# HopperLogger/HopperRender

Measured on AMD Instinct MI355X. Metric: interpolated frames/sec + ms/flow-calc, 2160p HDR, 1/2/4/8 MI355X, higher is better.
Workload: dtype u16

## Files before the change

### hopperrender_amd/csrc/hf_calc.hip

```cpp

#include "hf_ctx.h"

using namespace hfi;

namespace hfi {

int enqueue_flow_chain(const hf_ctx* const* cs, int n, hipStream_t s) {
    const hf_ctx* c = cs[0];
    const hf::Geom& g = c->g;
    const int iters = effective_iterations(c);
    bool any_big = false;
    for (int k = 0; k < iters; k++) any_big |= c->levels[k].window > 32;

    hf::FlowBatch a{};
    a.n = n;
    for (int i = 0; i < n; i++) {
        const hf_ctx* m = cs[i];
        hf::FlowStep& f = a.s[i];
        f.pp1 = m->pp[1].get();
        f.pp2 = m->pp[2].get();
        f.pl = m->pl;
        f.total_delta = m->d_total_delta;
        f.R = c->p.search_radius;
        f.delta_scalar = c->p.delta_scalar;
        f.neighbor_scalar = c->p.neighbor_scalar;
        f.delta_divisor = (uint32_t)(g.lh * g.lw * (g.hdr ? 6 : 10));
        f.sadtab = m->sadtab.get(); f.sad_nbx = m->sad_nbx; f.sad_nby = m->sad_nby;
        f.tables_base = m->tables.get(); f.sums_base = m->sums.get();
        f.counters = c->counters.get();
        f.still_count = m->still_count.get();
    }
    hf::FlowLevel none{};
    hf::PendingArgmin pending[hf::kMaxFlowBatch] = {};
    int step_index = 0;
    auto flush_pending = [&]() {
        if (!pending[0].active) return;
        hf::FlowBatch b = a;
        for (int i = 0; i < n; i++) {
            hf::FlowStep& f = b.s[i];
            const hf::PendingArgmin& p = pending[i];
            f.cur = p.lvl; f.prev = p.lvl_prev; f.axis = p.axis; f.capture_delta = p.capture_delta;
            f.sums = const_cast<uint32_t*>(p.sums); f.use_neighbors = p.use_neighbors; f.pend = hf::PendingArgmin{};
            pending[i] = hf::PendingArgmin{};
        }
        hf::launch_flow_big_argmin(g, b, s);
    };
    const bool lazy = !(c->cfg.flags & HF_FLAG_NO_LAZY_ARGMIN);
    bool tables_fresh = false;
    for (int k = 0; k < iters; k++) {
        const bool use_neighbors = k >= 4;
        if (use_neighbors) flush_pending();
        const bool small = c->levels[k].window <= 32;
        for (int axis = 0; axis < (small ? 1 : 2); axis++) {
            for (int i = 0; i < n; i++) {
                const hf_ctx* m = cs[i];
                hf::FlowStep& f = a.s[i];
                f.cur = m->levels[k];
                f.prev = k ? m->levels[k - 1] : none;
                f.prev2 = k > 1 ? m->levels[k - 2] : none;
                f.level_index = k;
                const hf::SadUse sad = hf::plan_sad_tables(m->levels.data(), k, c->tab_mode && m->sadtab);
                f.sad_write = sad.write; f.sad_read = sad.read;
                f.use_neighbors = use_neighbors;
                f.axis = axis;
                f.capture_delta = (k == 0 && axis == 0);
                f.pend = pending[i];
                if (!small) f.sums = m->sums.get() + (size_t)step_index * m->sums_stride;
                pending[i] = hf::PendingArgmin{};
            }
            if (a.s[0].sad_read && !tables_fresh)
                return fail(const_cast<hf_ctx*>(c), HF_ERR_STATE, "flow chain: level %d (window %d) would read SAD tables that level %d did not write", k, c->levels[k].window, k - 1);
            tables_fresh = a.s[0].sad_write != 0;
            if (small) {
                hf::launch_flow_level_small(g, a, s);
            } else {
                hf::launch_flow_big_partial(g, a, s);
                for (int i = 0; i < n; i++) {
                    const hf::FlowStep& f = a.s[i];
                    pending[i].active = 1; pending[i].axis = axis; pending[i].capture_delta = f.capture_delta;
                    pending[i].use_neighbors = f.use_neighbors;
                    pending[i].lvl = f.cur; pending[i].lvl_prev = f.prev; pending[i].sums = f.sums;
                }
                step_index++;
                if (!lazy || use_neighbors) flush_pending();
            }
        }
    }
    flush_pending();
    hf::BlurBatch bb{};
    bb.n = n;
    for (int i = 0; i < n; i++) {
        const hf_ctx* m = cs[i];
        bb.s[i].last = iters ? m->levels[iters - 1] : none;
        bb.s[i].blurred = m->blurred[0].get();
        bb.s[i].packed = m->blurred_xy[0].get();
        bb.s[i].zero = any_big ? m->sums.get() : nullptr;
        bb.s[i].still_count = m->still_count.get();
        bb.s[i].still_out = m->still_count ? m->d_total_delta + 1 : nullptr;
    }
    hf::launch_blur_flow(g, bb, c->cfg.blur_radius, (int)(c->sums_bytes / sizeof(uint32_t)), s);
    HF_HIP(const_cast<hf_ctx*>(c), hipGetLastError());
    return HF_OK;
}

bool choose_tab_mode(hf_ctx* const* cs, int n) {
    hf_ctx* l = cs[0];
    if (!l->sadtab) return false;
    if (l->cfg.flags & HF_FLAG_SAD_REUSE_ALWAYS) return true;
    if (n < 4) return false;
    float sum = 0.f;
    int have = 0;
    for (int i = 0; i < n; i++) {
        hf_ctx* m = cs[i];
        const uint32_t raw = m->h_total_delta ? ((volatile uint32_t*)m->h_total_delta.get())[1] : 0xFFFFFFFFu;
        int n32 = 0;
        for (const hf::FlowLevel& L : m->levels) if (L.window == 32) n32 = L.nwx * L.nwy;
        if (raw != 0xFFFFFFFFu && n32 > 0) {
            const float share = (float)raw / (float)n32;
            m->still_share = m->still_share < 0.f ? share : 0.5f * m->still_share + 0.5f * share;
        }
        if (m->still_share >= 0.f) { sum += m->still_share; have++; }
    }
    if (!have) return l->tab_mode;
    const float share = sum / (float)have;
    return l->tab_mode ? share >= 0.30f : share >= 0.45f;
// ... 450 lines not shown
```

### hopperrender_amd/csrc/hf_context.hip

```cpp

#include "hf_ctx.h"

using namespace hfi;

namespace {
thread_local std::string g_create_error;
}

namespace hfi {
std::shared_mutex g_capture_mutex;
std::atomic<int64_t> g_live[kLiveKinds];
}

namespace hfi {

int fail(hf_ctx* c, int code, const char* fmt, ...) {
    char buf[512];
    va_list ap;
    va_start(ap, fmt);
    vsnprintf(buf, sizeof(buf), fmt, ap);
    va_end(ap);
    std::string msg = std::string("[HopperRender] ") + buf;
    if (c) c->err = msg; else g_create_error = msg;
    return code;
// ... 149 lines not shown
    hf::Geom& g = c->g;
    g.hdr = cfg->is_hdr ? 1 : 0;
    g.H = cfg->frame_height;
    g.W = cfg->frame_width;
    g.in_stride = cfg->input_stride > 0 ? cfg->input_stride : g.W;
    g.out_stride = cfg->output_stride > 0 ? cfg->output_stride : g.W;
    g.rs = 0;
    while ((g.H >> g.rs) > cfg->max_calc_res) g.rs++;
    g.lw = (int)std::ceil((double)g.W / std::pow(2.0, g.rs));
    g.lh = (int)std::ceil((double)g.H / std::pow(2.0, g.rs));
    if (g.in_stride < g.W || g.out_stride < g.W) {
        delete c;
        return fail(nullptr, HF_ERR_INVALID_ARGUMENT, "hf_create: strides must be >= frame width");
    }
    if (((cfg->flags & HF_FLAG_PLANAR_IN) && (g.in_stride & 1)) || ((cfg->flags & HF_FLAG_PLANAR_OUT) && (g.out_stride & 1))) {
        delete c;
        return fail(nullptr, HF_ERR_INVALID_ARGUMENT, "hf_create: a planar side needs an even stride (input %d, output %d)", g.in_stride, g.out_stride);
    }
    if (c->cfg.blur_radius <= 0) c->cfg.blur_radius = 4;
    if (c->cfg.blur_radius > 64) { delete c; return fail(nullptr, HF_ERR_INVALID_ARGUMENT, "hf_create: blur_radius must be <= 64"); }
    c->p.delta_scalar = cfg->delta_scalar;
    c->p.neighbor_scalar = cfg->neighbor_scalar;
    c->p.black_level = cfg->black_level;
    c->p.white_level = cfg->white_level;
    c->p.search_radius = cfg->search_radius > 0 ? cfg->search_radius : kMinSearchRadius;
    c->p.frame_count = 0;
    if (c->p.search_radius < 2 || c->p.search_radius > kMaxSearchRadius) {
        delete c;
        return fail(nullptr, HF_ERR_INVALID_ARGUMENT, "hf_create: search_radius must be in [2, 16]");
    }

    const size_t bpp = g.hdr ? 2 : 1;
    c->in_bytes = bpp * ((size_t)g.H * g.in_stride + (size_t)(g.H / 2) * g.in_stride);
    c->out_bytes = bpp * ((size_t)g.H * g.out_stride + (size_t)(g.H / 2) * g.out_stride);
    c->plane_elems = (size_t)g.lw * g.lh;
    const int ws0 = initial_window(g.lw, g.lh);
    const int max_iters = ilog2(ws0);
    c->pl = hf::make_phase_layout(g, max_iters);
    {
        size_t elems = 0;
        for (int k = 0, w = ws0; k < max_iters; k++, w >>= 1) {
            hf::FlowLevel L{};
            L.window = w; L.log2w = ilog2(w);
            L.nwx = (g.lw + w - 1) / w; L.nwy = (g.lh + w - 1) / w;
            c->levels.push_back(L);
            elems += 2 * (size_t)L.nwx * L.nwy;
        }
        c->tables_bytes = (elems + 8) * sizeof(int16_t);
    }
    const size_t nwin_max = (size_t)((g.lw + 63) / 64) * ((g.lh + 63) / 64) + 1;
    c->sums_stride = nwin_max * 16;
    c->sums_bytes = (size_t)kMaxSteps * c->sums_stride * sizeof(uint32_t);
    c->sad_nbx = (g.lw + 1) / 2; c->sad_nby = (g.lh + 1) / 2;
    c->sadtab_bytes = (cfg->flags & HF_FLAG_NO_SAD_REUSE) ? 0 : 2 * (size_t)c->sad_nbx * c->sad_nby * 32;
    int rc = HF_OK;
    auto bail = [&](int code) { std::string e = c->err; hf_destroy(c); g_create_error = e; return code; };
    {
        const uint64_t required = 3 * c->in_bytes + 3 * c->pl.bytes + c->out_bytes + c->tables_bytes + c->sums_bytes + c->sadtab_bytes +
                                  2 * c->plane_elems * sizeof(int16_t) * 3 + 2 * c->plane_elems * sizeof(uint32_t);
        std::vector<hf_device_caps> caps((size_t)ndev);
        for (int d = 0; d < ndev; d++) {
            hipDeviceProp_t prop;
            if (hipGetDeviceProperties(&prop, d) != hipSuccess) { caps[(size_t)d] = hf_device_caps{}; continue; }
            caps[(size_t)d] = hf_device_caps{(uint64_t)prop.totalGlobalMem, (uint64_t)prop.sharedMemPerBlock, prop.maxThreadsPerBlock, prop.warpSize};
        }
        char why[384] = "";
        const int first = cfg->device_index >= 0 ? cfg->device_index : 0, last = cfg->device_index >= 0 ? cfg->device_index + 1 : ndev;
        int chosen = -1;
        for (int start = first; start < last && chosen < 0;) {
            const int rel = hf_select_device(caps.data() + start, last - start, required, why, sizeof(why));
            if (rel < 0) break;
            const int d = start + rel;
            size_t free_b = 0, total_b = 0;
            if (hipSetDevice(d) == hipSuccess && hipMemGetInfo(&free_b, &total_b) == hipSuccess && free_b >= required) { chosen = d; break; }
            snprintf(why, sizeof(why), "Not enough VRAM available! Required: %llu MB, Available: %llu MB", (unsigned long long)(required / 1024 / 1024),
                     (unsigned long long)(free_b / 1024 / 1024));
            start = d + 1;
        }
        if (chosen < 0) {
            fail(c, HF_ERR_NO_DEVICE, "Error in function detectDevices: no suitable HIP GPU found among device%s %d..%d! %s", last - first > 1 ? "s" : "",
                 first, last - 1, why);
            return bail(HF_ERR_NO_DEVICE);
        }
        c->device = chosen;
        c->cfg.device_index = chosen;
    }
    if ((rc = set_device(c))) return bail(rc);
#define HF_TRY(call) do { hipError_t _e = (call); if (_e != hipSuccess) { \
        fail(c, _e == hipErrorOutOfMemory ? HF_ERR_OUT_OF_MEMORY : HF_ERR_HIP, "HIP error %d (%s) in %s", (int)_e, hipGetErrorString(_e), #call); \
        return bail(_e == hipErrorOutOfMemory ? HF_ERR_OUT_OF_MEMORY : HF_ERR_HIP); } } while (0)
    HF_TRY(create_stream(c->own_stream));
    c->stream = c->own_stream.get();
    if (cfg->flags & HF_FLAG_DUAL_STREAM) {
        HF_TRY(create_stream(c->own_warp_stream));
        HF_TRY(create_event(c->ev_flow[0], hipEventDisableTiming));
        HF_TRY(create_event(c->ev_flow[1], hipEventDisableTiming));
    }
    c->warp_stream = c->own_warp_stream ? c->own_warp_stream.get() : c->stream;
    HF_TRY(create_event(c->ev_chain_done, hipEventDisableTiming));
    HF_TRY(create_event(c->ev_warps_done, hipEventDisableTiming));
    for (int i = 0; i < 3; i++) {
        HF_TRY(alloc_device(c->ring_store[i], c->in_bytes));
        c->ring[i] = c->ring_store[i].get();
        HF_TRY(alloc_device(c->pp[i], c->pl.bytes));
        HF_TRY(hipMemsetAsync(c->ring[i], 0, c->in_bytes, c->stream));
        HF_TRY(hipMemsetAsync(c->pp[i].get(), 0, c->pl.bytes, c->stream));
    }
// ... 354 lines not shown
```

### hopperrender_amd/csrc/hf_flow.hip

```cpp
#include <utility>
#include "hf_kernels.h"
#include "hf_phase_plane.h"

namespace hf {

thread_local LaunchObserver* t_launch_observer = nullptr;

namespace {

__device__ __forceinline__ int clampi(int v, int lo, int hi) { return min(max(v, lo), hi); }

__device__ __forceinline__ int rel_offset(int layer, int R) {
    const int d = layer - (R >> 1);
    return d > 0 ? d * d : -(d * d);
}

__device__ __forceinline__ int mirror_clamp(int p, int dim) {
    if (p >= dim) p = 2 * dim - p - 1; else if (p < 0) p = -p - 1;
    return clampi(p, 0, dim - 1);
}

template <typename E>
__global__ __launch_bounds__(256) void prep_phase_kernel(const PrepBatch batch, int H, int W, int S, PhaseLayout pl) {
    const E* __restrict__ f = (const E*)batch.frame[blockIdx.y];
// ... 458 lines not shown
        } else {
            const bool hi = (lane & M) != 0;
            const uint32_t send = hi ? v[k] : v[k + NV / 2];
            const uint32_t keep = hi ? v[k + NV / 2] : v[k];
            v[k] = keep + lane_xor<M>(send, lane);
        }
    }
}

struct Best { uint32_t sum; int cz; };
__device__ __forceinline__ void best_min(Best& b, uint32_t s, int cz) {
    if (s < b.sum || (s == b.sum && cz < b.cz)) { b.sum = s; b.cz = cz; }
}
template <int M>
__device__ __forceinline__ void best_xor(Best& b, int lane) {
    const uint32_t s = lane_xor<M>(b.sum, lane);
    const int c = (int)lane_xor<M>((uint32_t)b.cz, lane);
    best_min(b, s, c);
}
template <int M>
__device__ __forceinline__ uint32_t or_xor(uint32_t v, int lane) { return v | lane_xor<M>(v, lane); }

template <int G> struct Owned;
template <> struct Owned<64> { static constexpr int n = 1; };
template <> struct Owned<16> { static constexpr int n = 1; };
template <> struct Owned<4> { static constexpr int n = 4; };
template <> struct Owned<2> { static constexpr int n = 8; };
template <> struct Owned<1> { static constexpr int n = 16; };

template <int G, int XM = 1>
__device__ __forceinline__ int group_reduce(uint32_t* sad, int lane) {
    if constexpr (G == 1) {
        return 0;
    } else if constexpr (G == 2) {
        butterfly_level<16, XM>(sad, lane);
        return (lane & XM) ? 8 : 0;
    } else if constexpr (G == 64) {
        butterfly_level<16, 32>(sad, lane); butterfly_level<8, 16>(sad, lane);
        butterfly_level<4, 8>(sad, lane);   butterfly_level<2, 4>(sad, lane);
        sad[0] += lane_xor<2>(sad[0], lane);
        sad[0] += lane_xor<1>(sad[0], lane);
        return ((lane >> 5) & 1) * 8 + ((lane >> 4) & 1) * 4 + ((lane >> 3) & 1) * 2 + ((lane >> 2) & 1);
    } else if constexpr (G == 16) {
        butterfly_level<16, 8>(sad, lane); butterfly_level<8, 4>(sad, lane);
        butterfly_level<4, 2>(sad, lane);  butterfly_level<2, 1>(sad, lane);
        return ((lane >> 3) & 1) * 8 + ((lane >> 2) & 1) * 4 + ((lane >> 1) & 1) * 2 + (lane & 1);
    } else {
        static_assert(G == 4, "lane groups of 1, 2, 4, 16 or 64");
        butterfly_level<16, 2>(sad, lane); butterfly_level<8, 1>(sad, lane);
        return ((lane >> 1) & 1) * 8 + (lane & 1) * 4;
    }
}

template <int G, bool R16, int XM = 1>
__device__ __forceinline__ int group_argmin(const uint32_t* tot, int first, const FlowStep& a, int searched0,
                                            const NbPacked& nb, uint32_t npix, int cap_cz, bool want_cap, uint32_t& captured, int lane) {
    const int R = R16 ? 16 : a.R;
    Best b{0xFFFFFFFFu, 16};
    uint32_t cap = 0;
#pragma unroll
    for (int k = 0; k < Owned<G>::n; k++) {
        const int cz = first + k;
        if (cz < R) {
            const int cand = (int)(int16_t)(searched0 + rel_offset(cz, R));
            const uint32_t sum = (tot[k] << a.delta_scalar) + npix * window_bias(cand, a.use_neighbors, nb, a.neighbor_scalar);
            if (k == 0 || sum < b.sum) { b.sum = sum; b.cz = cz; }
            if (cz == cap_cz) cap = sum;
        }
    }
    if (G == 64) { best_xor<4>(b, lane); best_xor<8>(b, lane); best_xor<16>(b, lane); best_xor<32>(b, lane); }
    else if (G == 16) { best_xor<1>(b, lane); best_xor<2>(b, lane); best_xor<4>(b, lane); best_xor<8>(b, lane); }
    else if (G == 4) { best_xor<1>(b, lane); best_xor<2>(b, lane); }
    else if (G == 2) { best_xor<XM>(b, lane); }
    if (want_cap) {
        if (G == 64) { cap = or_xor<4>(cap, lane); cap = or_xor<8>(cap, lane); cap = or_xor<16>(cap, lane); cap = or_xor<32>(cap, lane); }
        else if (G == 16) { cap = or_xor<1>(cap, lane); cap = or_xor<2>(cap, lane); cap = or_xor<4>(cap, lane); cap = or_xor<8>(cap, lane); }
        else if (G == 4) { cap = or_xor<1>(cap, lane); cap = or_xor<2>(cap, lane); }
        else if (G == 2) { cap = or_xor<XM>(cap, lane); }
        captured = cap;
    }
    return b.cz;
}

__device__ __forceinline__ int resolve_pending(const Geom& g, const FlowStep& a, int px, int py, int lane, bool origin_leader) {
    const PendingArgmin& p = a.pend;
    const int wx = px >> p.lvl.log2w, wy = py >> p.lvl.log2w, w = wy * p.lvl.nwx + wx;
    const int x0 = wx << p.lvl.log2w, y0 = wy << p.lvl.log2w;
    int searched0 = 0;
    if (p.lvl_prev.tx) searched0 = table_at(p.axis ? p.lvl_prev.ty : p.lvl_prev.tx, p.lvl_prev, x0, y0);
    const uint32_t npix = (uint32_t)((min(g.lw, x0 + p.lvl.window) - x0) * (min(g.lh, y0 + p.lvl.window) - y0));
    const int cz = lane & 15;
    Best b{0xFFFFFFFFu, 16};
    uint32_t mine = 0;
    HF_DBG_CHECK(wx >= 0 && wy >= 0 && wx < p.lvl.nwx && wy < p.lvl.nwy, 104);
    if (cz < a.R) {
        const int cand = (int)(int16_t)(searched0 + rel_offset(cz, a.R));
        mine = (p.sums[w * 16 + cz] << a.delta_scalar) + npix * ((uint32_t)(cand < 0 ? -cand : cand) & 0xFFFFu);
        b.sum = mine; b.cz = cz;
    }
    best_xor<1>(b, lane); best_xor<2>(b, lane); best_xor<4>(b, lane); best_xor<8>(b, lane);
    const int value = (int)(int16_t)(searched0 + rel_offset(b.cz, a.R));
    if (p.capture_delta && w == 0) {
        uint32_t cap = cz == (a.R >> 1) - 1 ? mine : 0u;
        cap = or_xor<1>(cap, lane); cap = or_xor<2>(cap, lane); cap = or_xor<4>(cap, lane); cap = or_xor<8>(cap, lane);
        if (origin_leader) *a.total_delta = cap / a.delta_divisor;
    }
    if (origin_leader) (p.axis ? p.lvl.ty : p.lvl.tx)[w] = (int16_t)value;
    return value;
}

struct FlowPtrs {
    const uint32_t *pp1, *pp2;
    int16_t* tables;
    uint32_t *sums, *total_delta, *sadtab, *still_count;
};
struct FlowBatchArgs {
    int n;
    FastDiv tiles, tiles_x;
    FlowStep common;
    FlowPtrs m[kMaxFlowBatch];
};
static_assert(sizeof(FlowBatchArgs) + sizeof(Geom) <= 4096, "kernel arguments of a batched chain launch");
static FlowBatchArgs pack_batch(const FlowBatch& b, int tiles_x, int tiles_y) {
    FlowBatchArgs k;
    k.n = b.n;
    const uint64_t max_v = (uint64_t)tiles_x * tiles_y * b.n + 8;
    k.tiles = make_fastdiv((uint32_t)(tiles_x * tiles_y), max_v); k.tiles_x = make_fastdiv((uint32_t)tiles_x, (uint64_t)tiles_x * tiles_y);
    k.common = b.s[0];
// ... 143 lines not shown
            if ((lane & 3) == 0) s_part[axis][wave][first] = sad[0];
            __syncthreads();
            sad[0] = s_part[axis][0][first] + s_part[axis][1][first] + s_part[axis][2][first] + s_part[axis][3][first];
        }
        const int best = group_argmin<G, R16, M::XM>(sad, first, a, off[axis], axis ? wc.nby : wc.nbx, wc.npix, cap_cz,
                                                      axis == 0 && a.capture_delta, captured, lane);
        off[axis] = (int)(int16_t)(off[axis] + rel_offset(best, R));
    }

    const bool leader = WS == 32 ? tid == 0 : G == 2 ? (lane & M::XM) == 0 : (lane & (G - 1)) == 0;
    HF_DBG_CHECK(!win_in || (wx >= 0 && wy >= 0 && wx < a.cur.nwx && wy < a.cur.nwy), 105);
    if (win_in && leader) {
        a.cur.tx[wy * a.cur.nwx + wx] = (int16_t)off[0];
        a.cur.ty[wy * a.cur.nwx + wx] = (int16_t)off[1];
        if (a.capture_delta && wx == 0 && wy == 0) *a.total_delta = captured / a.delta_divisor;
        if (WS == 32 && a.still_count && off[0] == wc.ox && off[1] == wc.oy) atomicAdd(a.still_count, 1u);
    }
}


template <int G, int XM>
__device__ __forceinline__ int packed_reduce(uint32_t* v, uint32_t* tot, int lane) {
    if constexpr (G == 64) {
        butterfly_level<8, 32>(v, lane); butterfly_level<4, 16>(v, lane); butterfly_level<2, 8>(v, lane);
        const uint32_t w = v[0] + lane_xor<4>(v[0], lane);
        uint32_t t = (lane & 4) ? w >> 16 : w & 0xFFFFu;
        t += lane_xor<2>(t, lane);
        t += lane_xor<1>(t, lane);
        tot[0] = t;
        return ((lane >> 5) & 1) * 8 + ((lane >> 4) & 1) * 4 + ((lane >> 3) & 1) * 2 + ((lane >> 2) & 1);
    } else if constexpr (G == 16) {
        butterfly_level<8, 8>(v, lane); butterfly_level<4, 4>(v, lane); butterfly_level<2, 2>(v, lane);
        const uint32_t w = v[0] + lane_xor<1>(v[0], lane);
        tot[0] = (lane & 1) ? w >> 16 : w & 0xFFFFu;
        return ((lane >> 3) & 1) * 8 + ((lane >> 2) & 1) * 4 + ((lane >> 1) & 1) * 2 + (lane & 1);
    } else if constexpr (G == 4) {
        butterfly_level<8, 2>(v, lane); butterfly_level<4, 1>(v, lane);
        tot[0] = v[0] & 0xFFFFu; tot[1] = v[0] >> 16; tot[2] = v[1] & 0xFFFFu; tot[3] = v[1] >> 16;
        return ((lane >> 1) & 1) * 8 + (lane & 1) * 4;
    } else {
        static_assert(G == 2, "windows of 64, 16, 4 or 2 lanes");
        butterfly_level<8, XM>(v, lane);
#pragma unroll
        for (int j = 0; j < 4; j++) { tot[2 * j] = v[j] & 0xFFFFu; tot[2 * j + 1] = v[j] >> 16; }
        return (lane & XM) ? 8 : 0;
    }
}

__device__ __forceinline__ void unpack_u16x8(const flow_v4& q, uint32_t* o) {
    o[0] = q.x & 0xFFFFu; o[1] = q.x >> 16; o[2] = q.y & 0xFFFFu; o[3] = q.y >> 16;
    o[4] = q.z & 0xFFFFu; o[5] = q.z >> 16; o[6] = q.w & 0xFFFFu; o[7] = q.w >> 16;
}

constexpr int kTabGroups = 2;
template <int WS, bool SPLIT, bool ROWS1>
__device__ __forceinline__ void flow_level_tab_body(const Geom& g, const FlowStep& a, int cx0, int cy, int lx, int ly, int tid, const TileId& tile,
                                                    uint32_t (*s_part)[4][16], [[maybe_unused]] uint32_t* s_rows) {
    using M = typename MapSel<WS, ROWS1>::type;
    constexpr int PX = M::PX, G = M::G, NR = M::NR, NOWN = Owned<G>::n;
    constexpr int NV = (PX == 4 && NR == 2) ? 4 : (PX == 2 && NR == 1) ? 1 : 2;
    const int wave = tid >> 6, lane = tid & 63;
    const int wx = cx0 >> a.cur.log2w, wy = cy >> a.cur.log2w;

    WinConst wc = load_win_const(g, a, wx, wy, false);
    const int nblk = a.sad_nbx * a.sad_nby;
    const int blk = (cy >> 1) * a.sad_nbx + (cx0 >> 1) + ((PX == 4 && NR == 1) ? (cy & 1) : 0);
    HF_DBG_CHECK(blk >= 0 && blk + (PX == 4 && NR == 2 ? 1 : 0) < nblk, 110);
    flow_v4* const tab0 = (flow_v4*)a.sadtab + (size_t)blk * 2 + ((PX == 2 && NR == 1 && (lane & M::XM)) ? 1 : 0);
    const size_t tab_axis = (size_t)nblk * 2;
    bool zx = false, zy = false;
    flow_v4 pre[2][NV];
    if (WS < 32 && a.sad_read) {
        int gx = 0, gy = 0;
        if (a.prev2.tx) {
            gx = table_at(a.prev2.tx, a.prev2, wx << a.cur.log2w, wy << a.cur.log2w);
            gy = table_at(a.prev2.ty, a.prev2, wx << a.cur.log2w, wy << a.cur.log2w);
        }
#pragma unroll
        for (int ax = 0; ax < 2; ax++)
#pragma unroll
            for (int v = 0; v < NV; v++) pre[ax][v] = tab0[ax * tab_axis + v];
        zx = wc.ox == gx; zy = wc.oy == gy;
    }
    if (a.pend.active) {
        const int tx0 = tile.tx * M::TW, ty0 = tile.ty * M::TH;
        const bool leader = tid == 0 && (tx0 & (a.pend.lvl.window - 1)) == 0 && (ty0 & (a.pend.lvl.window - 1)) == 0;
        const int v = resolve_pending(g, a, tx0, ty0, lane, leader);
        if (a.pend.axis) wc.oy = v; else wc.ox = v;
    }
    const int cap_cz = 7;
    uint32_t captured = 0;
    int off[2] = {wc.ox, wc.oy};

#pragma unroll
    for (int axis = 0; axis < 2; axis++) {
        bool reuse = zy && (axis == 0 ? zx : off[0] == wc.ox);
        if constexpr (G == 64) reuse = __builtin_amdgcn_readfirstlane((int)reuse) != 0;
        if (a.counters) {
            const bool lead = WS == 32 ? tid == 0 : G == 2 ? (lane & M::XM) == 0 : (lane & (G - 1)) == 0;
            const uint64_t mw = __builtin_amdgcn_ballot_w64(lead), mr = __builtin_amdgcn_ballot_w64(lead && reuse);
            if (lane == 0 && mw) {
                uint32_t* const c = a.counters + kCounterLevels + 4 * (a.level_index & 15) + 2 * axis;
                atomicAdd(c, (uint32_t)__builtin_popcountll(mw));
                if (mr) atomicAdd(c + 1, (uint32_t)__builtin_popcountll(mr));
            }
        }
        flow_v4* const tab = tab0 + axis * tab_axis;
        uint32_t tot[NOWN];
        int first = 0;
        if constexpr (PX == 4 && NR == 1) {
            uint32_t W[8];
            if (!reuse) {
                Strip<PX> strip[NR];
#pragma unroll
                for (int r = 0; r < NR; r++) strip[r] = load_strip<PX, true>(g, a, cx0, cy + r);
                uint32_t p[16];
#pragma unroll
                for (int cz = 0; cz < 16; cz++) p[cz] = 0u;
                bool from_lds = false;
                if constexpr (WS == 16 && SPLIT) {
                    if (axis == 1) from_lds = ysads_tile_try<16, 4, 1, true, kTabGroups>(p, g, a, strip[0].ref, off[0], off[1], cx0, cy, lane, s_rows);
                } else if constexpr (WS == 8 && SPLIT) {
                    if (axis == 1) from_lds = ysads_win8_try<true, kTabGroups>(p, g, a, strip[0].ref, off[0], off[1], cx0, cy, lane, s_rows);
                } else if constexpr (WS == 32) {
                    if (axis == 1) from_lds = ysads_tile_try<32, 8, 4, true, kTabGroups>(p, g, a, strip[0].ref, off[0], off[1], cx0 - lx, cy - ly, tid, s_rows);
                }
                if (!from_lds) strip_sads<4, G == 64, true, true, true, kTabGroups>(p, g, a, strip[0], off[0], off[1], axis);
                const uint32_t selw = (cy & 1) ? 0x07060302u : 0x05040100u;
#pragma unroll
                for (int j = 0; j < 8; j++) {
                    const uint32_t q0 = p[2 * j] + lane_xor<M::RM>(p[2 * j], lane);
                    const uint32_t q1 = p[2 * j + 1] + lane_xor<M::RM>(p[2 * j + 1], lane);
                    W[j] = __builtin_amdgcn_perm(q1, q0, selw);
                }
                if (a.sad_write) { tab[0] = flow_v4{W[0], W[1], W[2], W[3]}; tab[1] = flow_v4{W[4], W[5], W[6], W[7]}; }
            } else {
                const flow_v4 lo = pre[axis][0], hi = pre[axis][1];
                W[0] = lo.x; W[1] = lo.y; W[2] = lo.z; W[3] = lo.w; W[4] = hi.x; W[5] = hi.y; W[6] = hi.z; W[7] = hi.w;
            }
            first = packed_reduce<G, M::XM>(W, tot, lane);
        } else if constexpr (PX == 4) {
            uint32_t V[8];
            if (!reuse) {
                Strip<PX> strip[NR];
#pragma unroll
                for (int r = 0; r < NR; r++) strip[r] = load_strip<PX, true>(g, a, cx0, cy + r);
                uint32_t p[16];
#pragma unroll
                for (int cz = 0; cz < 16; cz++) p[cz] = 0u;
#pragma unroll
                for (int r = 0; r < NR; r++) strip_sads<4, false, true, true, true, kTabGroups>(p, g, a, strip[r], off[0], off[1], axis);
                uint32_t W0[8], W1[8];
#pragma unroll
                for (int j = 0; j < 8; j++) {
                    W0[j] = __builtin_amdgcn_perm(p[2 * j + 1], p[2 * j], 0x05040100u);
                    W1[j] = __builtin_amdgcn_perm(p[2 * j + 1], p[2 * j], 0x07060302u);
                    V[j] = W0[j] + W1[j];
                }
                if (a.sad_write) {
                    tab[0] = flow_v4{W0[0], W0[1], W0[2], W0[3]}; tab[1] = flow_v4{W0[4], W0[5], W0[6], W0[7]};
                    tab[2] = flow_v4{W1[0], W1[1], W1[2], W1[3]}; tab[3] = flow_v4{W1[4], W1[5], W1[6], W1[7]};
                }
            } else {
                const flow_v4 a0 = pre[axis][0], a1 = pre[axis][1], b0 = pre[axis][2 % NV], b1 = pre[axis][3 % NV];
                V[0] = a0.x + b0.x; V[1] = a0.y + b0.y; V[2] = a0.z + b0.z; V[3] = a0.w + b0.w;
                V[4] = a1.x + b1.x; V[5] = a1.y + b1.y; V[6] = a1.z + b1.z; V[7] = a1.w + b1.w;
            }
            first = packed_reduce<G, M::XM>(V, tot, lane);
        } else if constexpr (NR == 2) {
            if (!reuse) {
                Strip<PX> strip[NR];
#pragma unroll
                for (int r = 0; r < NR; r++) strip[r] = load_strip<PX, true>(g, a, cx0, cy + r);
#pragma unroll
                for (int cz = 0; cz < 16; cz++) tot[cz] = 0u;
#pragma unroll
                for (int r = 0; r < NR; r++) strip_sads<PX, false, true, false, true, kTabGroups>(tot, g, a, strip[r], off[0], off[1], axis);
            } else {
                unpack_u16x8(pre[axis][0], tot); unpack_u16x8(pre[axis][1 % NV], tot + 8);
            }
        } else {
            if (!reuse) {
                Strip<PX> strip[NR];
#pragma unroll
                for (int r = 0; r < NR; r++) strip[r] = load_strip<PX, true>(g, a, cx0, cy + r);
                uint32_t sad[16];
#pragma unroll
                for (int cz = 0; cz < 16; cz++) sad[cz] = 0u;
                strip_sads<PX, false, true, false, true, kTabGroups>(sad, g, a, strip[0], off[0], off[1], axis);
                butterfly_level<16, M::XM>(sad, lane);
#pragma unroll
                for (int k = 0; k < 8; k++) tot[k] = sad[k];
            } else {
                unpack_u16x8(pre[axis][0], tot);
            }
            first = (lane & M::XM) ? 8 : 0;
        }
        if constexpr (WS == 32) {
            if ((lane & 3) == 0) s_part[axis][wave][first] = tot[0];
            __syncthreads();
            tot[0] = s_part[axis][0][first] + s_part[axis][1][first] + s_part[axis][2][first] + s_part[axis][3][first];
        }
        const int best = group_argmin<G, true, M::XM>(tot, first, a, off[axis], axis ? wc.nby : wc.nbx, wc.npix, cap_cz,
                                                      axis == 0 && a.capture_delta, captured, lane);
        off[axis] = (int)(int16_t)(off[axis] + rel_offset(best, 16));
    }

    const bool leader = WS == 32 ? tid == 0 : G == 2 ? (lane & M::XM) == 0 : (lane & (G - 1)) == 0;
    HF_DBG_CHECK(wx >= 0 && wy >= 0 && wx < a.cur.nwx && wy < a.cur.nwy, 105);
    if (leader) {
        a.cur.tx[wy * a.cur.nwx + wx] = (int16_t)off[0];
        a.cur.ty[wy * a.cur.nwx + wx] = (int16_t)off[1];
        if (WS == 32 && a.still_count && off[0] == wc.ox && off[1] == wc.oy) atomicAdd(a.still_count, 1u);
        if (a.capture_delta && wx == 0 && wy == 0) *a.total_delta = captured / a.delta_divisor;
    }
}

template <bool FULL, bool R16, int NH>
__device__ __forceinline__ void flow_level32_wave_body(const Geom& g, const FlowStep& a, const TileId& tile, [[maybe_unused]] uint32_t* s_rows) {
    using M = Map<32>;
    const int R = R16 ? 16 : a.R;
    const int lane = (int)threadIdx.x;
    int lx, ly;
    M::at(lane, lx, ly);
    const int tx0 = tile.tx * M::TW, ty0 = tile.ty * M::TH;
    const int cx0 = tx0 + lx;
    const int wx = tx0 >> a.cur.log2w, wy = ty0 >> a.cur.log2w;
    WinConst wc = load_win_const(g, a, wx, wy, false);
    if (a.pend.active) {
        const bool leader = lane == 0 && (tx0 & (a.pend.lvl.window - 1)) == 0 && (ty0 & (a.pend.lvl.window - 1)) == 0;
        const int v = resolve_pending(g, a, tx0, ty0, lane, leader);
        if (a.pend.axis) wc.oy = v; else wc.ox = v;
    }
    const int cap_cz = (R >> 1) - 1;
    uint32_t captured = 0;
    int off[2] = {wc.ox, wc.oy};
#pragma unroll
    for (int axis = 0; axis < 2; axis++) {
        uint32_t sad[16];
#pragma unroll
        for (int cz = 0; cz < 16; cz++) sad[cz] = 0u;
        bool staged = false;
        if constexpr (FULL) if (axis == 1) {
            staged = ytile_can_stage<32>(g, a, __builtin_amdgcn_readfirstlane(off[1]), ty0);
            if (staged) with_rs(g.rs, [&](auto RS) { ystage_copy<decltype(RS)::value, 32, 8, 1>(a, __builtin_amdgcn_readfirstlane(off[0]), __builtin_amdgcn_readfirstlane(off[1]), tx0, ty0, lane, s_rows); });
        }
#pragma unroll 1
        for (int v = 0; v < 4; v++) {
            const Strip<4> strip = load_strip<4, FULL>(g, a, cx0, ty0 + ly + 8 * v);
            if (staged) with_rs(g.rs, [&](auto RS) { ystage_sads<decltype(RS)::value, 32, 8, 1, false, NH>(sad, a, strip.ref, __builtin_amdgcn_readfirstlane(off[0]), v * 64 + lane, s_rows); });
            else strip_sads<4, true, FULL, false, R16, NH>(sad, g, a, strip, off[0], off[1], axis);
        }
        const int first = group_reduce<64, 1>(sad, lane);
        const int best = group_argmin<64, R16, 1>(sad, first, a, off[axis], axis ? wc.nby : wc.nbx, wc.npix, cap_cz,
                                                  axis == 0 && a.capture_delta, captured, lane);
        off[axis] = (int)(int16_t)(off[axis] + rel_offset(best, R));
    }
    HF_DBG_CHECK(wx >= 0 && wy >= 0 && wx < a.cur.nwx && wy < a.cur.nwy, 105);
    if (lane == 0) {
        a.cur.tx[wy * a.cur.nwx + wx] = (int16_t)off[0];
        a.cur.ty[wy * a.cur.nwx + wx] = (int16_t)off[1];
        if (a.capture_delta && wx == 0 && wy == 0) *a.total_delta = captured / a.delta_divisor;
        if (a.still_count && off[0] == wc.ox && off[1] == wc.oy) atomicAdd(a.still_count, 1u);
    }
}

__device__ __forceinline__ void flow_level32_wave_tab_body(const Geom& g, const FlowStep& a, const TileId& tile, [[maybe_unused]] uint32_t* s_rows) {
    using M = Map<32>;
    const int lane = (int)threadIdx.x;
    int lx, ly;
    M::at(lane, lx, ly);
    const int tx0 = tile.tx * M::TW, ty0 = tile.ty * M::TH;
    const int cx0 = tx0 + lx, cy_0 = ty0 + ly;
    const int wx = tx0 >> a.cur.log2w, wy = ty0 >> a.cur.log2w;
    WinConst wc = load_win_const(g, a, wx, wy, false);
    const int nblk = a.sad_nbx * a.sad_nby;
    const int blk = (cy_0 >> 1) * a.sad_nbx + (cx0 >> 1) + (cy_0 & 1);
    HF_DBG_CHECK(blk >= 0 && blk + 12 * a.sad_nbx < nblk, 110);
    flow_v4* const tab0 = (flow_v4*)a.sadtab + (size_t)blk * 2;
    const size_t tab_axis = (size_t)nblk * 2, tab_round = (size_t)a.sad_nbx * 8;
    if (a.pend.active) {
        const bool leader = lane == 0 && (tx0 & (a.pend.lvl.window - 1)) == 0 && (ty0 & (a.pend.lvl.window - 1)) == 0;
        const int v = resolve_pending(g, a, tx0, ty0, lane, leader);
        if (a.pend.axis) wc.oy = v; else wc.ox = v;
    }
    const int cap_cz = 7;
    uint32_t captured = 0;
    int off[2] = {wc.ox, wc.oy};
    const uint32_t selw = (cy_0 & 1) ? 0x07060302u : 0x05040100u;
#pragma unroll
    for (int axis = 0; axis < 2; axis++) {
        if (a.counters && lane == 0) atomicAdd(a.counters + kCounterLevels + 4 * (a.level_index & 15) + 2 * axis, 1u);
        flow_v4* const tab = tab0 + axis * tab_axis;
        bool staged = false;
        if (axis == 1) {
            staged = ytile_can_stage<32>(g, a, __builtin_amdgcn_readfirstlane(off[1]), ty0);
            if (staged) with_rs(g.rs, [&](auto RS) { ystage_copy<decltype(RS)::value, 32, 8, 1>(a, __builtin_amdgcn_readfirstlane(off[0]), __builtin_amdgcn_readfirstlane(off[1]), tx0, ty0, lane, s_rows); });
        }
        uint32_t total = 0;
        int first = 0;
#pragma unroll 1
        for (int v = 0; v < 4; v++) {
            const Strip<4> strip = load_strip<4, true>(g, a, cx0, cy_0 + 8 * v);
            uint32_t p[16];
#pragma unroll
            for (int cz = 0; cz < 16; cz++) p[cz] = 0u;
            if (staged) with_rs(g.rs, [&](auto RS) { ystage_sads<decltype(RS)::value, 32, 8, 1, true, kTabGroups>(p, a, strip.ref, __builtin_amdgcn_readfirstlane(off[0]), v * 64 + lane, s_rows); });
            else strip_sads<4, true, true, true, true, kTabGroups>(p, g, a, strip, off[0], off[1], axis);
            uint32_t W[8];
#pragma unroll
            for (int j = 0; j < 8; j++) {
                const uint32_t q0 = p[2 * j] + lane_xor<M::RM>(p[2 * j], lane);
                const uint32_t q1 = p[2 * j + 1] + lane_xor<M::RM>(p[2 * j + 1], lane);
                W[j] = __builtin_amdgcn_perm(q1, q0, selw);
            }
            if (a.sad_write) { tab[v * tab_round] = flow_v4{W[0], W[1], W[2], W[3]}; tab[v * tab_round + 1] = flow_v4{W[4], W[5], W[6], W[7]}; }
            uint32_t t1[1];
            first = packed_reduce<64, 1>(W, t1, lane);
            total += t1[0];
        }
        const uint32_t tot[1] = {total};
        const int best = group_argmin<64, true, 1>(tot, first, a, off[axis], axis ? wc.nby : wc.nbx, wc.npix, cap_cz,
                                                   axis == 0 && a.capture_delta, captured, lane);
        off[axis] = (int)(int16_t)(off[axis] + rel_offset(best, 16));
    }
    HF_DBG_CHECK(wx >= 0 && wy >= 0 && wx < a.cur.nwx && wy < a.cur.nwy, 105);
    if (lane == 0) {
        a.cur.tx[wy * a.cur.nwx + wx] = (int16_t)off[0];
        a.cur.ty[wy * a.cur.nwx + wx] = (int16_t)off[1];
        if (a.still_count && off[0] == wc.ox && off[1] == wc.oy) atomicAdd(a.still_count, 1u);
        if (a.capture_delta && wx == 0 && wy == 0) *a.total_delta = captured / a.delta_divisor;
    }
}

template <bool TABK>
__global__ __launch_bounds__(64) void flow_level32_wave_kernel(const Geom g, const FlowBatchArgs batch) {
    const TileId tile = decode_tile<1>(batch, (g.lw + 31) / 32, (g.lh + 31) / 32);
    if (!tile.valid) return;
    const FlowStep a = member_step(batch, tile.pair);
    extern __shared__ __attribute__((aligned(16))) uint32_t s_rows[];
    const bool full = a.R == 16 && (tile.tx + 1) * 32 <= g.lw && (tile.ty + 1) * 32 <= g.lh;
    if constexpr (TABK) {
        if (full) flow_level32_wave_tab_body(g, a, tile, s_rows);
        else flow_level32_wave_body<false, true, kTabGroups>(g, a, tile, s_rows);
    }
    else if (full) flow_level32_wave_body<true, true, 1>(g, a, tile, s_rows);
    else if (a.R == 16) flow_level32_wave_body<false, true, 1>(g, a, tile, s_rows);
    else flow_level32_wave_body<false, false, 1>(g, a, tile, s_rows);
}

template <int WS, bool SPLIT, bool ROWS1 = false, bool TABK = false>
__global__ __launch_bounds__(SPLIT ? 64 : 256) void flow_level_small_kernel(const Geom g, const FlowBatchArgs batch) {
    using M = typename MapSel<WS, ROWS1>::type;
    const TileId tile = decode_tile<SPLIT ? M::WAVES : 1>(batch, (g.lw + M::TW - 1) / M::TW, (g.lh + M::TH - 1) / M::TH);
    if (!tile.valid) return;
    const FlowStep a = member_step(batch, tile.pair);
    static_assert(!SPLIT || WS <= 16, "a 32x32 window is shared by the four waves of a workgroup");
    __shared__ uint32_t s_part[SPLIT ? 1 : 2][4][16];
    extern __shared__ __attribute__((aligned(16))) uint32_t s_rows[];
    const bool full = a.R == 16 && (tile.tx + 1) * M::TW <= g.lw && (tile.ty + 1) * M::TH <= g.lh;
    if constexpr (TABK) {
        const bool tab = full && (M::TW == 32 || ((tile.tx * M::TW) | 31) < g.lw);
        if (tab) {
            const int tid = SPLIT ? (int)(tile.wave * 64 + threadIdx.x) : (int)threadIdx.x;
            int lx, ly;
            M::at(tid, lx, ly);
            flow_level_tab_body<WS, SPLIT, ROWS1>(g, a, tile.tx * M::TW + lx, tile.ty * M::TH + ly, lx, ly, tid, tile, s_part, s_rows);
        }
        else if (full) flow_level_small_body<WS, SPLIT, true, ROWS1, true, kTabGroups>(g, a, tile, s_part, s_rows);
        else flow_level_small_body<WS, SPLIT, false, ROWS1, true, kTabGroups>(g, a, tile, s_part, s_rows);
    }
    else if (full) flow_level_small_body<WS, SPLIT, true, ROWS1>(g, a, tile, s_part, s_rows);
    else if (a.R == 16) flow_level_small_body<WS, SPLIT, false, ROWS1, true>(g, a, tile, s_part, s_rows);
    else flow_level_small_body<WS, SPLIT, false, ROWS1>(g, a, tile, s_part, s_rows);
}
// ... 225 lines not shown
```

### hopperrender_amd/csrc/hf_kernels.h

```cpp
#pragma once
#include <hip/hip_runtime.h>
#ifdef __HIPCC__
#include <hip/hip_ext.h>
#endif
#include <stdint.h>
#include "hf_launch_plan.h"

#ifdef HF_DEBUG_BOUNDS
#ifdef __HIPCC__
namespace hf { namespace {
__device__ unsigned int g_dbg_bounds[5];
__device__ __forceinline__ void dbg_bounds_record(int site, int line) {
    if (atomicAdd(&g_dbg_bounds[0], 1u) == 0u) {
        g_dbg_bounds[1] = (unsigned)site; g_dbg_bounds[2] = (unsigned)blockIdx.x; g_dbg_bounds[3] = (unsigned)threadIdx.x; g_dbg_bounds[4] = (unsigned)line;
    }
}
} }
#define HF_DBG_CHECK(cond, site) do { if (!(cond)) ::hf::dbg_bounds_record((site), __LINE__); } while (0)
#else
#define HF_DBG_CHECK(cond, site) do { } while (0)
#endif
#else
#define HF_DBG_CHECK(cond, site) do { } while (0)
#endif

namespace hf {

struct LaunchObserver {
    virtual bool next(const char* kernel_name, hipEvent_t* start, hipEvent_t* stop) = 0;
protected:
    ~LaunchObserver() = default;
};
extern thread_local LaunchObserver* t_launch_observer;

#ifdef __HIPCC__
#define HF_LAUNCH(NAME, KERNEL, GRID, BLOCK, LDS, STREAM, ...)                                                     \
    do {                                                                                                            \
        hipEvent_t hf_e0_ = nullptr, hf_e1_ = nullptr;                                                              \
        if (::hf::t_launch_observer && ::hf::t_launch_observer->next((NAME), &hf_e0_, &hf_e1_))                    \
            hipExtLaunchKernelGGL(KERNEL, GRID, BLOCK, LDS, STREAM, hf_e0_, hf_e1_, 0, __VA_ARGS__);                \
        else                                                                                                        \
            hipLaunchKernelGGL(KERNEL, GRID, BLOCK, LDS, STREAM, __VA_ARGS__);                                      \
    } while (0)
#endif

#ifdef __HIPCC__
__device__ __forceinline__ uint32_t fastdiv(uint32_t u, const FastDiv f) { return f.magic ? __umulhi(u, f.magic) : f.d > 1 ? u / f.d : u; }
#endif

constexpr int kCounterWarp = 0, kCounterLevels = 8, kCounterWords = 8 + 4 * 16;
struct PendingArgmin {
    int active;
    int axis;
    int capture_delta;
    int use_neighbors;
    FlowLevel lvl;
    FlowLevel lvl_prev;
    const uint32_t* sums;
};

struct FlowStep {
    const uint32_t* pp1;
    const uint32_t* pp2;
    PhaseLayout pl;
    FlowLevel cur, prev;
    uint32_t* sums;
    uint32_t* total_delta;
    int axis;
    int R;
    int use_neighbors;
    int delta_scalar, neighbor_scalar;
    int capture_delta;
    uint32_t delta_divisor;
    PendingArgmin pend;
    FlowLevel prev2;
    uint32_t* sadtab;
    int sad_nbx, sad_nby;
    int sad_read;
    int sad_write;
    int y_rows_lds;
    uint32_t* still_count;
    uint32_t* counters;
    int level_index;
    int16_t* tables_base;
    uint32_t* sums_base;
};

struct FlowBatch {
    int n;
    FlowStep s[kMaxFlowBatch];
};
struct BlurItem {
    FlowLevel last;
    int16_t* blurred;
    uint32_t* packed;
    uint32_t* zero;
    uint32_t* still_count;
    uint32_t* still_out;
};
struct BlurBatch {
    int n;
    BlurItem s[kMaxFlowBatch];
};

struct PrepBatch {
    int n;
    const void* frame[kMaxFlowBatch];
    uint32_t* pp[kMaxFlowBatch];
};
void launch_prep_frames(const Geom& g, const PhaseLayout& pl, const PrepBatch& b, hipStream_t stream);
void launch_prep_grid(const Geom& g, const PhaseLayout& pl, const PrepBatch& b, hipStream_t stream);
void launch_flow_level_small(const Geom& g, const FlowBatch& b, hipStream_t stream);
// ... 74 lines not shown
```

Baseline: 100,100.

## Store per-window SAD sum pyramid so finer levels read precomputed totals

While the coarse flow levels reduce their SAD candidates, they now write partial sums for 16-, 8- and 4-pixel windows into a pyramid appended to the SAD table buffer. Finer levels then load their per-window totals straight from that pyramid instead of re-reading raw 2x2 block tables and re-running the packed lane reduction. The butterfly reduction order is rearranged so owner lanes line up with pyramid slots, and the argmin reduction skips xor stages for duplicated lanes. This costs extra global writes and a larger table allocation, and adds a host-side check that the level above actually wrote the sums being read.

```diff
diff --git a/hopperrender_amd/csrc/hf_calc.hip b/hopperrender_amd/csrc/hf_calc.hip
--- a/hopperrender_amd/csrc/hf_calc.hip
+++ b/hopperrender_amd/csrc/hf_calc.hip
@@ -47,6 +47,7 @@
     };
     const bool lazy = !(c->cfg.flags & HF_FLAG_NO_LAZY_ARGMIN);
     bool tables_fresh = false;
+    int pyramid_below = 0;
     for (int k = 0; k < iters; k++) {
         const bool use_neighbors = k >= 4;
         if (use_neighbors) flush_pending();
@@ -70,7 +71,11 @@
             }
             if (a.s[0].sad_read && !tables_fresh)
                 return fail(const_cast<hf_ctx*>(c), HF_ERR_STATE, "flow chain: level %d (window %d) would read SAD tables that level %d did not write", k, c->levels[k].window, k - 1);
+            const int ws = c->levels[k].window;
+            if (a.s[0].sad_read && ws >= 4 && ws <= 16 && ws >= pyramid_below)
+                return fail(const_cast<hf_ctx*>(c), HF_ERR_STATE, "flow chain: level %d (window %d) would read window sums that level %d did not write", k, ws, k - 1);
             tables_fresh = a.s[0].sad_write != 0;
+            pyramid_below = a.s[0].sad_write ? ws : 0;
             if (small) {
                 hf::launch_flow_level_small(g, a, s);
             } else {
diff --git a/hopperrender_amd/csrc/hf_context.hip b/hopperrender_amd/csrc/hf_context.hip
--- a/hopperrender_amd/csrc/hf_context.hip
+++ b/hopperrender_amd/csrc/hf_context.hip
@@ -225,7 +225,7 @@
     c->sums_stride = nwin_max * 16;
     c->sums_bytes = (size_t)kMaxSteps * c->sums_stride * sizeof(uint32_t);
     c->sad_nbx = (g.lw + 1) / 2; c->sad_nby = (g.lh + 1) / 2;
-    c->sadtab_bytes = (cfg->flags & HF_FLAG_NO_SAD_REUSE) ? 0 : 2 * (size_t)c->sad_nbx * c->sad_nby * 32;
+    c->sadtab_bytes = (cfg->flags & HF_FLAG_NO_SAD_REUSE) ? 0 : hf::sad_pyramid(c->sad_nbx, c->sad_nby).words * sizeof(uint32_t);
     int rc = HF_OK;
     auto bail = [&](int code) { std::string e = c->err; hf_destroy(c); g_create_error = e; return code; };
     {
diff --git a/hopperrender_amd/csrc/hf_flow.hip b/hopperrender_amd/csrc/hf_flow.hip
--- a/hopperrender_amd/csrc/hf_flow.hip
+++ b/hopperrender_amd/csrc/hf_flow.hip
@@ -534,7 +534,7 @@
     }
 }
 
-template <int G, bool R16, int XM = 1>
+template <int G, bool R16, int XM = 1, int DUP = 3>
 __device__ __forceinline__ int group_argmin(const uint32_t* tot, int first, const FlowStep& a, int searched0,
                                             const NbPacked& nb, uint32_t npix, int cap_cz, bool want_cap, uint32_t& captured, int lane) {
     const int R = R16 ? 16 : a.R;
@@ -550,12 +550,26 @@
             if (cz == cap_cz) cap = sum;
         }
     }
-    if (G == 64) { best_xor<4>(b, lane); best_xor<8>(b, lane); best_xor<16>(b, lane); best_xor<32>(b, lane); }
+    if constexpr (G == 64) {
+        if constexpr (!(DUP & 1)) best_xor<1>(b, lane);
+        if constexpr (!(DUP & 2)) best_xor<2>(b, lane);
+        if constexpr (!(DUP & 4)) best_xor<4>(b, lane);
+        if constexpr (!(DUP & 8)) best_xor<8>(b, lane);
+        if constexpr (!(DUP & 16)) best_xor<16>(b, lane);
+        if constexpr (!(DUP & 32)) best_xor<32>(b, lane);
+    }
     else if (G == 16) { best_xor<1>(b, lane); best_xor<2>(b, lane); best_xor<4>(b, lane); best_xor<8>(b, lane); }
     else if (G == 4) { best_xor<1>(b, lane); best_xor<2>(b, lane); }
     else if (G == 2) { best_xor<XM>(b, lane); }
     if (want_cap) {
-        if (G == 64) { cap = or_xor<4>(cap, lane); cap = or_xor<8>(cap, lane); cap = or_xor<16>(cap, lane); cap = or_xor<32>(cap, lane); }
+        if constexpr (G == 64) {
+            if constexpr (!(DUP & 1)) cap = or_xor<1>(cap, lane);
+            if constexpr (!(DUP & 2)) cap = or_xor<2>(cap, lane);
+            if constexpr (!(DUP & 4)) cap = or_xor<4>(cap, lane);
+            if constexpr (!(DUP & 8)) cap = or_xor<8>(cap, lane);
+            if constexpr (!(DUP & 16)) cap = or_xor<16>(cap, lane);
+            if constexpr (!(DUP & 32)) cap = or_xor<32>(cap, lane);
+        }
         else if (G == 16) { cap = or_xor<1>(cap, lane); cap = or_xor<2>(cap, lane); cap = or_xor<4>(cap, lane); cap = or_xor<8>(cap, lane); }
         else if (G == 4) { cap = or_xor<1>(cap, lane); cap = or_xor<2>(cap, lane); }
         else if (G == 2) { cap = or_xor<XM>(cap, lane); }
@@ -805,6 +819,29 @@
     o[4] = q.z & 0xFFFFu; o[5] = q.z >> 16; o[6] = q.w & 0xFFFFu; o[7] = q.w >> 16;
 }
 
+template <int WS> struct PyrStages;
+template <> struct PyrStages<32> { static constexpr int M1 = 16, M2 = 8, M3 = 32, M4 = 1, DUP = 2 | 4; };
+template <> struct PyrStages<16> { static constexpr int M1 = 8, M2 = 4, M3 = 16, M4 = 1, DUP = 2 | 32; };
+template <> struct PyrStages<8> { static constexpr int M1 = 4, M2 = 2, M3 = 8, M4 = 1, DUP = 0; };
+template <int WS>
+__device__ __forceinline__ int pyramid_owner(int lane) {
+    using S = PyrStages<WS>;
+    return ((lane & S::M1) ? 8 : 0) + ((lane & S::M2) ? 4 : 0) + ((lane & S::M3) ? 2 : 0) + ((lane & S::M4) ? 1 : 0);
+}
+template <int WS>
+__device__ __forceinline__ void pyramid_reduce(uint32_t* v, uint32_t& t, int lane, bool write, uint32_t* p4e, [[maybe_unused]] uint32_t* p8e) {
+    using S = PyrStages<WS>;
+    butterfly_level<8, S::M1>(v, lane); butterfly_level<4, S::M2>(v, lane);
+    const int pair = ((lane & S::M1) ? 4 : 0) + ((lane & S::M2) ? 2 : 0);
+    if (write) *(uint2*)(p4e + pair) = make_uint2(v[0], v[1]);
+    butterfly_level<2, S::M3>(v, lane);
+    const uint32_t w = v[0] + lane_xor<S::M4>(v[0], lane);
+    if constexpr (WS > 8) {
+        if (write && !(lane & S::M4)) p8e[pair + ((lane & S::M3) ? 1 : 0)] = w;
+    }
+    t = (lane & S::M4) ? w >> 16 : w & 0xFFFFu;
+}
+
 constexpr int kTabGroups = 2;
 template <int WS, bool SPLIT, bool ROWS1>
 __device__ __forceinline__ void flow_level_tab_body(const Geom& g, const FlowStep& a, int cx0, int cy, int lx, int ly, int tid, const TileId& tile,
@@ -821,8 +858,14 @@
     HF_DBG_CHECK(blk >= 0 && blk + (PX == 4 && NR == 2 ? 1 : 0) < nblk, 110);
     flow_v4* const tab0 = (flow_v4*)a.sadtab + (size_t)blk * 2 + ((PX == 2 && NR == 1 && (lane & M::XM)) ? 1 : 0);
     const size_t tab_axis = (size_t)nblk * 2;
+    const SadPyramid py = sad_pyramid(a.sad_nbx, a.sad_nby);
+    uint32_t* const p4e = a.sadtab + py.p4 + ((size_t)(cy >> 2) * py.n4x + (cx0 >> 2)) * 8;
+    uint32_t* const p8e = a.sadtab + py.p8 + ((size_t)(cy >> 3) * py.n8x + (cx0 >> 3)) * 8;
+    HF_DBG_CHECK((cx0 >> 2) < py.n4x && (cy >> 2) < py.n4y && (cx0 >> 3) < py.n8x && (cy >> 3) < py.n8y, 111);
+    [[maybe_unused]] __shared__ uint32_t s_half[WS == 32 ? 2 : 1][4][2][16];
     bool zx = false, zy = false;
     flow_v4 pre[2][NV];
+    uint32_t own[2][4];
     if (WS < 32 && a.sad_read) {
         int gx = 0, gy = 0;
         if (a.prev2.tx) {
@@ -830,9 +873,28 @@
             gy = table_at(a.prev2.ty, a.prev2, wx << a.cur.log2w, wy << a.cur.log2w);
         }
 #pragma unroll
-        for (int ax = 0; ax < 2; ax++)
-#pragma unroll
-            for (int v = 0; v < NV; v++) pre[ax][v] = tab0[ax * tab_axis + v];
+        for (int ax = 0; ax < 2; ax++) {
+            if constexpr (WS == 16) {
+                HF_DBG_CHECK(wx < py.n16x && wy < py.n16y, 112);
+                own[ax][0] = a.sadtab[py.p16 + ax * py.p16_axis + ((size_t)wy * py.n16x + wx) * 16 + pyramid_owner<16>(lane)];
+            } else if constexpr (WS == 8) {
+                HF_DBG_CHECK(wx < py.n8x && wy < py.n8y, 112);
+                own[ax][0] = ((const uint16_t*)(a.sadtab + py.p8 + ax * py.p8_axis + ((size_t)wy * py.n8x + wx) * 8))[pyramid_owner<8>(lane)];
+            } else if constexpr (WS == 4) {
+                HF_DBG_CHECK(wx < py.n4x && wy < py.n4y, 112);
+                const uint32_t* const e = a.sadtab + py.p4 + ax * py.p4_axis + ((size_t)wy * py.n4x + wx) * 8;
+                if constexpr (G == 2) {
+                    const flow_v4 q = *(const flow_v4*)(e + ((lane & M::XM) ? 4 : 0));
+                    own[ax][0] = q.x; own[ax][1] = q.y; own[ax][2] = q.z; own[ax][3] = q.w;
+                } else {
+                    const uint2 q = *(const uint2*)(e + ((lane & 2) ? 4 : 0) + ((lane & 1) ? 2 : 0));
+                    own[ax][0] = q.x; own[ax][1] = q.y;
+                }
+            } else {
+#pragma unroll
+                for (int v = 0; v < NV; v++) pre[ax][v] = tab0[ax * tab_axis + v];
+            }
+        }
         zx = wc.ox == gx; zy = wc.oy == gy;
     }
     if (a.pend.active) {
@@ -887,11 +949,27 @@
                     W[j] = __builtin_amdgcn_perm(q1, q0, selw);
                 }
                 if (a.sad_write) { tab[0] = flow_v4{W[0], W[1], W[2], W[3]}; tab[1] = flow_v4{W[4], W[5], W[6], W[7]}; }
-            } else {
-                const flow_v4 lo = pre[axis][0], hi = pre[axis][1];
-                W[0] = lo.x; W[1] = lo.y; W[2] = lo.z; W[3] = lo.w; W[4] = hi.x; W[5] = hi.y; W[6] = hi.z; W[7] = hi.w;
-            }
-            first = packed_reduce<G, M::XM>(W, tot, lane);
+                if constexpr (WS >= 8) {
+                    uint32_t t;
+                    pyramid_reduce<WS>(W, t, lane, a.sad_write != 0, p4e + axis * py.p4_axis, p8e + axis * py.p8_axis);
+                    if constexpr (WS == 16) { t += lane_xor<2>(t, lane); t += lane_xor<32>(t, lane); }
+                    if constexpr (WS == 32) {
+                        t += lane_xor<2>(t, lane);
+                        if ((lane & 2) == 0) s_half[axis][wave][(lane >> 2) & 1][pyramid_owner<32>(lane)] = t;
+                        t += lane_xor<4>(t, lane);
+                    }
+                    tot[0] = t;
+                    first = pyramid_owner<WS>(lane);
+                } else {
+                    first = packed_reduce<G, M::XM>(W, tot, lane);
+                }
+            } else if constexpr (WS == 16 || WS == 8) {
+                tot[0] = own[axis][0];
+                first = pyramid_owner<WS>(lane);
+            } else if constexpr (WS == 4) {
+                tot[0] = own[axis][0] & 0xFFFFu; tot[1] = own[axis][0] >> 16; tot[2] = own[axis][1] & 0xFFFFu; tot[3] = own[axis][1] >> 16;
+                first = ((lane >> 1) & 1) * 8 + (lane & 1) * 4;
+            }
         } else if constexpr (PX == 4) {
             uint32_t V[8];
             if (!reuse) {
@@ -914,12 +992,12 @@
                     tab[0] = flow_v4{W0[0], W0[1], W0[2], W0[3]}; tab[1] = flow_v4{W0[4], W0[5], W0[6], W0[7]};
                     tab[2] = flow_v4{W1[0], W1[1], W1[2], W1[3]}; tab[3] = flow_v4{W1[4], W1[5], W1[6], W1[7]};
                 }
+                first = packed_reduce<G, M::XM>(V, tot, lane);
             } else {
-                const flow_v4 a0 = pre[axis][0], a1 = pre[axis][1], b0 = pre[axis][2 % NV], b1 = pre[axis][3 % NV];
-                V[0] = a0.x + b0.x; V[1] = a0.y + b0.y; V[2] = a0.z + b0.z; V[3] = a0.w + b0.w;
-                V[4] = a1.x + b1.x; V[5] = a1.y + b1.y; V[6] = a1.z + b1.z; V[7] = a1.w + b1.w;
-            }
-            first = packed_reduce<G, M::XM>(V, tot, lane);
+#pragma unroll
+                for (int j = 0; j < 4; j++) { tot[2 * j] = own[axis][j] & 0xFFFFu; tot[2 * j + 1] = own[axis][j] >> 16; }
+                first = (lane & M::XM) ? 8 : 0;
+            }
         } else if constexpr (NR == 2) {
             if (!reuse) {
                 Strip<PX> strip[NR];
@@ -950,12 +1028,19 @@
             first = (lane & M::XM) ? 8 : 0;
         }
         if constexpr (WS == 32) {
-            if ((lane & 3) == 0) s_part[axis][wave][first] = tot[0];
+            if ((lane & PyrStages<32>::DUP) == 0) s_part[axis][wave][first] = tot[0];
             __syncthreads();
             tot[0] = s_part[axis][0][first] + s_part[axis][1][first] + s_part[axis][2][first] + s_part[axis][3][first];
-        }
-        const int best = group_argmin<G, true, M::XM>(tot, first, a, off[axis], axis ? wc.nby : wc.nbx, wc.npix, cap_cz,
-                                                      axis == 0 && a.capture_delta, captured, lane);
+            if (a.sad_write && tid < 64) {
+                const int h = tid >> 5, s = (tid >> 4) & 1, cz = tid & 15;
+                const int w16 = ((cy - ly) >> 4) + h, v16 = ((cx0 - lx) >> 4) + s;
+                HF_DBG_CHECK(v16 < py.n16x && w16 < py.n16y, 113);
+                a.sadtab[py.p16 + axis * py.p16_axis + ((size_t)w16 * py.n16x + v16) * 16 + cz] = s_half[axis][2 * h][s][cz] + s_half[axis][2 * h + 1][s][cz];
+            }
+        }
+        constexpr int DUP = (WS == 32 || WS == 16) ? PyrStages<WS == 32 ? 32 : 16>::DUP : 3;
+        const int best = group_argmin<G, true, M::XM, DUP>(tot, first, a, off[axis], axis ? wc.nby : wc.nbx, wc.npix, cap_cz,
+                                                           axis == 0 && a.capture_delta, captured, lane);
         off[axis] = (int)(int16_t)(off[axis] + rel_offset(best, 16));
     }
 
@@ -1032,6 +1117,10 @@
     HF_DBG_CHECK(blk >= 0 && blk + 12 * a.sad_nbx < nblk, 110);
     flow_v4* const tab0 = (flow_v4*)a.sadtab + (size_t)blk * 2;
     const size_t tab_axis = (size_t)nblk * 2, tab_round = (size_t)a.sad_nbx * 8;
+    const SadPyramid py = sad_pyramid(a.sad_nbx, a.sad_nby);
+    const int first = pyramid_owner<32>(lane);
+    HF_DBG_CHECK((cx0 >> 2) < py.n4x && ((cy_0 + 24) >> 2) < py.n4y && (cx0 >> 3) < py.n8x && ((cy_0 + 24) >> 3) < py.n8y &&
+                 (cx0 >> 4) < py.n16x && (ty0 >> 4) + 1 < py.n16y, 111);
     if (a.pend.active) {
         const bool leader = lane == 0 && (tx0 & (a.pend.lvl.window - 1)) == 0 && (ty0 & (a.pend.lvl.window - 1)) == 0;
         const int v = resolve_pending(g, a, tx0, ty0, lane, leader);
@@ -1050,8 +1139,10 @@
             staged = ytile_can_stage<32>(g, a, __builtin_amdgcn_readfirstlane(off[1]), ty0);
             if (staged) with_rs(g.rs, [&](auto RS) { ystage_copy<decltype(RS)::value, 32, 8, 1>(a, __builtin_amdgcn_readfirstlane(off[0]), __builtin_amdgcn_readfirstlane(off[1]), tx0, ty0, lane, s_rows); });
         }
-        uint32_t total = 0;
-        int first = 0;
+        uint32_t* const p4e = a.sadtab + py.p4 + axis * py.p4_axis + ((size_t)(cy_0 >> 2) * py.n4x + (cx0 >> 2)) * 8;
+        uint32_t* const p8e = a.sadtab + py.p8 + axis * py.p8_axis + ((size_t)(cy_0 >> 3) * py.n8x + (cx0 >> 3)) * 8;
+        uint32_t* const p16e = a.sadtab + py.p16 + axis * py.p16_axis + ((size_t)(ty0 >> 4) * py.n16x + (cx0 >> 4)) * 16 + first;
+        uint32_t total = 0, half = 0;
 #pragma unroll 1
         for (int v = 0; v < 4; v++) {
             const Strip<4> strip = load_strip<4, true>(g, a, cx0, cy_0 + 8 * v);
@@ -1068,12 +1159,18 @@
                 W[j] = __builtin_amdgcn_perm(q1, q0, selw);
             }
             if (a.sad_write) { tab[v * tab_round] = flow_v4{W[0], W[1], W[2], W[3]}; tab[v * tab_round + 1] = flow_v4{W[4], W[5], W[6], W[7]}; }
-            uint32_t t1[1];
-            first = packed_reduce<64, 1>(W, t1, lane);
-            total += t1[0];
-        }
+            uint32_t t;
+            pyramid_reduce<32>(W, t, lane, a.sad_write != 0, p4e + (size_t)v * 2 * py.n4x * 8, p8e + (size_t)v * py.n8x * 8);
+            half += t + lane_xor<2>(t, lane);
+            if (v & 1) {
+                if (a.sad_write && (lane & 2) == 0) p16e[(size_t)(v >> 1) * py.n16x * 16] = half;
+                total += half;
+                half = 0;
+            }
+        }
+        total += lane_xor<4>(total, lane);
         const uint32_t tot[1] = {total};
-        const int best = group_argmin<64, true, 1>(tot, first, a, off[axis], axis ? wc.nby : wc.nbx, wc.npix, cap_cz,
+        const int best = group_argmin<64, true, 1, PyrStages<32>::DUP>(tot, first, a, off[axis], axis ? wc.nby : wc.nbx, wc.npix, cap_cz,
                                                    axis == 0 && a.capture_delta, captured, lane);
         off[axis] = (int)(int16_t)(off[axis] + rel_offset(best, 16));
     }
diff --git a/hopperrender_amd/csrc/hf_kernels.h b/hopperrender_amd/csrc/hf_kernels.h
--- a/hopperrender_amd/csrc/hf_kernels.h
+++ b/hopperrender_amd/csrc/hf_kernels.h
@@ -58,6 +58,21 @@
     FlowLevel lvl_prev;
     const uint32_t* sums;
 };
+
+struct SadPyramid {
+    int n16x, n16y, n8x, n8y, n4x, n4y;
+    size_t blocks_axis, p16, p16_axis, p8, p8_axis, p4, p4_axis, words;
+};
+constexpr SadPyramid sad_pyramid(int nbx, int nby) {
+    SadPyramid p{};
+    p.n4x = (nbx + 1) >> 1; p.n4y = (nby + 1) >> 1; p.n8x = (nbx + 3) >> 2; p.n8y = (nby + 3) >> 2; p.n16x = (nbx + 7) >> 3; p.n16y = (nby + 7) >> 3;
+    p.blocks_axis = (size_t)nbx * nby * 8;
+    p.p16 = (2 * p.blocks_axis + 15) & ~(size_t)15; p.p16_axis = (size_t)p.n16x * p.n16y * 16;
+    p.p8 = p.p16 + 2 * p.p16_axis;                  p.p8_axis = (size_t)p.n8x * p.n8y * 8;
+    p.p4 = p.p8 + 2 * p.p8_axis;                    p.p4_axis = (size_t)p.n4x * p.n4y * 8;
+    p.words = p.p4 + 2 * p.p4_axis;
+    return p;
+}
 
 struct FlowStep {
     const uint32_t* pp1;
```

Result: no change. 99990 (-0.1%).
